# edouardoyallon/acco

Hardware: NVIDIA H100
Metric: tokens/sec (device-timed, max over ranks) Llama ACCO bf16 sharded-Adam, 8x1024 tokens per GPU per micro-batch (higher is better)
Workload: dtype bf16

## Files before the change

acco_b200/csrc/attention_wgmma.cu:

```cuda
#include <cuda.h>
#include <cuda_bf16.h>
#include <cuda_runtime.h>
#include <math.h>
#include <stdint.h>

#include "wgmma.cuh"

namespace acco_attn {

using namespace acco_tc;

constexpr int HD = 64;
constexpr int LDS = HD + 8;
constexpr float LOG2E = 1.4426950408889634f;
constexpr float LN2 = 0.6931471805599453f;

typedef __nv_bfloat16 bf16;

__device__ __forceinline__ uint32_t pack2(float a, float b) {
    __nv_bfloat162 h = __floats2bfloat162_rn(a, b);
    return *reinterpret_cast<uint32_t*>(&h);
}
__device__ __forceinline__ uint32_t ld32(const bf16* p) { return *reinterpret_cast<const uint32_t*>(p); }

__device__ __forceinline__ void mma16816(float (&c)[4], const uint32_t (&a)[4], uint32_t b0, uint32_t b1) {
    asm volatile("mma.sync.aligned.m16n8k16.row.col.f32.bf16.bf16.f32 {%0,%1,%2,%3}, {%4,%5,%6,%7}, {%8,%9}, {%0,%1,%2,%3};"
                 : "+f"(c[0]), "+f"(c[1]), "+f"(c[2]), "+f"(c[3])
                 : "r"(a[0]), "r"(a[1]), "r"(a[2]), "r"(a[3]), "r"(b0), "r"(b1));
}

template <int NB, int KB>
__device__ __forceinline__ void warp_mma_ss(float (&acc)[NB][4], const bf16* A, const bf16* B, int lane) {
    const int g = lane >> 2, t = lane & 3;
#pragma unroll
    for (int kb = 0; kb < KB; ++kb) {
        uint32_t a[4];
        const bf16* a0 = A + g * LDS + kb * 16 + 2 * t;
        a[0] = ld32(a0); a[1] = ld32(a0 + 8 * LDS); a[2] = ld32(a0 + 8); a[3] = ld32(a0 + 8 * LDS + 8);
#pragma unroll
        for (int nb = 0; nb < NB; ++nb) {
            const bf16* b = B + (nb * 8 + g) * LDS + kb * 16 + 2 * t;
            mma16816(acc[nb], a, ld32(b), ld32(b + 8));
        }
    }
}
template <int NB>
__device__ __forceinline__ void warp_mma_rs(float (&acc)[NB][4], const float (&p)[8][4], const bf16* B, int lane) {
    const int g = lane >> 2, t = lane & 3;
#pragma unroll
    for (int kb = 0; kb < 4; ++kb) {
        uint32_t a[4];
        a[0] = pack2(p[2 * kb][0], p[2 * kb][1]);
        a[1] = pack2(p[2 * kb][2], p[2 * kb][3]);
        a[2] = pack2(p[2 * kb + 1][0], p[2 * kb + 1][1]);
        a[3] = pack2(p[2 * kb + 1][2], p[2 * kb + 1][3]);
#pragma unroll
        for (int nb = 0; nb < NB; ++nb) {
            const bf16* b = B + (nb * 8 + g) * LDS + kb * 16 + 2 * t;
            mma16816(acc[nb], a, ld32(b), ld32(b + 8));
        }
    }
}

__device__ __forceinline__ void load_tile(bf16* dst, const bf16* src, long long ld, int rows, int valid, int tid, int nthr) {
    for (int i = tid; i < rows * 8; i += nthr) {
        const int r = i >> 3, c = (i & 7) * 8;
        uint4 v = make_uint4(0, 0, 0, 0);
        if (r < valid) v = *reinterpret_cast<const uint4*>(src + (long long)r * ld + c);
        *reinterpret_cast<uint4*>(dst + r * LDS + c) = v;
    }
}
__device__ __forceinline__ void load_tile_t(bf16* dst, const bf16* src, long long ld, int rows, int tid, int nthr) {
    for (int i = tid; i < rows * 8; i += nthr) {
        const int r = i >> 3, c = (i & 7) * 8;
        const uint4 v = *reinterpret_cast<const uint4*>(src + (long long)r * ld + c);
        const bf16* e = reinterpret_cast<const bf16*>(&v);
#pragma unroll
        for (int j = 0; j < 8; ++j) dst[(c + j) * LDS + r] = e[j];
    }
}

__device__ __forceinline__ bool visible(int q, int kv, int window) { return kv <= q && kv > q - window; }

struct FwdParams {
    CUtensorMap map_q;
    CUtensorMap map_k;
    CUtensorMap map_v;
    bf16* o;
    long long ld_o;
    float* lse;
    int B, S, Hq, Hk, window;
    float scale;
    const int* seg;
};

constexpr int FWD_Q = 128, FWD_KV = 64, FWD_THREADS = 256;
constexpr int FWD_TILE_KV = FWD_KV * HD * 2;
constexpr int FWD_SMEM = FWD_Q * HD * 2 + 2 * 2 * FWD_TILE_KV + 1024  + 64 ;

__device__ __forceinline__ void wgmma_m64n64k16_rs_tb(float (&d)[32], const uint32_t (&a)[4], uint64_t db) {
    asm volatile(
        "{\n\t.reg .pred p;\n\tsetp.ne.b32 p, %37, 0;\n\twgmma.mma_async.sync.aligned.m64n64k16.f32.bf16.bf16 "
        "{%0,%1,%2,%3,%4,%5,%6,%7,%8,%9,%10,%11,%12,%13,%14,%15,%16,%17,%18,%19,%20,%21,%22,%23,%24,%25,%26,%27,%28,%29,%30,%31}, "
        "{%32,%33,%34,%35}, %36, p, 1, 1, 1;\n\t}"
        : "+f"(d[0]), "+f"(d[1]), "+f"(d[2]), "+f"(d[3]), "+f"(d[4]), "+f"(d[5]), "+f"(d[6]), "+f"(d[7]), "+f"(d[8]), "+f"(d[9]), "+f"(d[10]),
          "+f"(d[11]), "+f"(d[12]), "+f"(d[13]), "+f"(d[14]), "+f"(d[15]), "+f"(d[16]), "+f"(d[17]), "+f"(d[18]), "+f"(d[19]), "+f"(d[20]),
          "+f"(d[21]), "+f"(d[22]), "+f"(d[23]), "+f"(d[24]), "+f"(d[25]), "+f"(d[26]), "+f"(d[27]), "+f"(d[28]), "+f"(d[29]), "+f"(d[30]),
          "+f"(d[31])
        : "r"(a[0]), "r"(a[1]), "r"(a[2]), "r"(a[3]), "l"(db), "r"(1));
}

template <bool kSeg>
__global__ void __launch_bounds__(FWD_THREADS) attn_fwd_kernel(const __grid_constant__ FwdParams P) {
    extern __shared__ uint8_t smem_raw[];
    uint8_t* smem = (uint8_t*)(((uintptr_t)smem_raw + 1023) & ~(uintptr_t)1023);
    uint8_t* sQ = smem;
    uint8_t* sKV = smem + FWD_Q * HD * 2;
    uint64_t* full = (uint64_t*)(sKV + 2 * 2 * FWD_TILE_KV);
    const int qb = blockIdx.x, h = blockIdx.y, b = blockIdx.z;
    const int hk = h / (P.Hq / P.Hk);
    const int tid = threadIdx.x, wg = tid >> 7, warp = (tid >> 5) & 3, lane = tid & 31, g = lane >> 2, t = lane & 3;
    const int q0 = qb * FWD_Q;
    const int row0 = b * P.S;
    int lo_key = max(0, q0 - P.window + 1);
    if constexpr (kSeg) lo_key = max(lo_key, P.seg[row0 + q0]);
    const int j_lo = lo_key / FWD_KV, j_hi = (q0 + FWD_Q - 1) / FWD_KV;
    auto issue = [&](int j) {
        const int s = (j - j_lo) & 1;
        mbar_expect_tx(&full[s], 2 * FWD_TILE_KV);
        tma_load_2d(&P.map_k, &full[s], sKV + s * 2 * FWD_TILE_KV, hk * HD, row0 + j * FWD_KV);
        tma_load_2d(&P.map_v, &full[s], sKV + s * 2 * FWD_TILE_KV + FWD_TILE_KV, hk * HD, row0 + j * FWD_KV);
    };
    if (tid == 0) {
        mbar_init(&full[0], 1);
        mbar_init(&full[1], 1);
        mbar_init(&full[2], 1);
        asm volatile("fence.mbarrier_init.release.cluster;" ::: "memory");
        mbar_expect_tx(&full[2], FWD_Q * HD * 2);
        tma_load_2d(&P.map_q, &full[2], sQ, h * HD, row0 + q0);
        issue(j_lo);
        if (j_lo + 1 <= j_hi) issue(j_lo + 1);
    }
    __syncthreads();
    mbar_wait(&full[2], 0);
    const float c = P.scale * LOG2E;
    float m_run[2] = {-INFINITY, -INFINITY}, l_run[2] = {0.f, 0.f};
    float o[32];
#pragma unroll
    for (int i = 0; i < 32; ++i) o[i] = 0.f;
    const int wq_lo = q0 + wg * 64, wq_hi = wq_lo + 63;
    const int qr[2] = {wq_lo + warp * 16 + g, wq_lo + warp * 16 + g + 8};
    int sg[2] = {0, 0}, wseg = 0;
    if constexpr (kSeg) {
        sg[0] = P.seg[row0 + qr[0]];
        sg[1] = P.seg[row0 + qr[1]];
        wseg = P.seg[row0 + wq_lo];
    }
    const uint32_t q_addr = smem_u32(sQ) + (uint32_t)(wg * 8192);
    for (int j = j_lo; j <= j_hi; ++j) {
        const int kv0 = j * FWD_KV, s = (j - j_lo) & 1;
        mbar_wait(&full[s], (uint32_t)(((j - j_lo) >> 1) & 1));
        if (!(kv0 > wq_hi || kv0 + FWD_KV - 1 <= wq_lo - P.window || (kSeg && kv0 + FWD_KV - 1 < wseg))) {
            const uint32_t k_addr = smem_u32(sKV + s * 2 * FWD_TILE_KV), v_addr = k_addr + FWD_TILE_KV;
            float sc[32];
#pragma unroll
            for (int i = 0; i < 32; ++i) sc[i] = 0.f;
            wgmma_fence();
#pragma unroll
            for (int k = 0; k < HD / 16; ++k)
                wgmma_m64n64k16<0, 0>(sc, make_smem_desc(q_addr + k * 32, 1, 1024 >> 4), make_smem_desc(k_addr + k * 32, 1, 1024 >> 4), 1u);
            wgmma_commit();
            wgmma_wait<0>();
            reg_fence(sc);
            float mx[2] = {-INFINITY, -INFINITY};
#pragma unroll
            for (int nb = 0; nb < 8; ++nb)
#pragma unroll
                for (int e = 0; e < 4; ++e) {
                    const int kv = kv0 + nb * 8 + 2 * t + (e & 1), r = e >> 1;
                    const float v = visible(qr[r], kv, P.window) && (!kSeg || kv >= sg[r]) ? sc[4 * nb + e] * c : -INFINITY;
                    sc[4 * nb + e] = v;
                    mx[r] = fmaxf(mx[r], v);
                }
#pragma unroll
            for (int r = 0; r < 2; ++r) {
                mx[r] = fmaxf(mx[r], __shfl_xor_sync(0xffffffffu, mx[r], 1));
                mx[r] = fmaxf(mx[r], __shfl_xor_sync(0xffffffffu, mx[r], 2));
            }
            float alpha[2], base[2], rs[2] = {0.f, 0.f};
#pragma unroll
            for (int r = 0; r < 2; ++r) {
                const float m_new = fmaxf(m_run[r], mx[r]);
                base[r] = m_new == -INFINITY ? 0.f : m_new;
                alpha[r] = exp2f(m_run[r] - base[r]);
                m_run[r] = m_new;
            }
#pragma unroll
            for (int i = 0; i < 32; ++i) {
                const int r = (i >> 1) & 1;
                const float p = exp2f(sc[i] - base[r]);
                sc[i] = p;
                rs[r] += p;
            }
#pragma unroll
            for (int r = 0; r < 2; ++r) {
                rs[r] += __shfl_xor_sync(0xffffffffu, rs[r], 1);
                rs[r] += __shfl_xor_sync(0xffffffffu, rs[r], 2);
                l_run[r] = l_run[r] * alpha[r] + rs[r];
            }
#pragma unroll
            for (int i = 0; i < 32; ++i) o[i] *= alpha[(i >> 1) & 1];
            wgmma_fence();
#pragma unroll
            for (int kk = 0; kk < FWD_KV / 16; ++kk) {
                uint32_t a[4];
                a[0] = pack2(sc[8 * kk + 0], sc[8 * kk + 1]);
                a[1] = pack2(sc[8 * kk + 2], sc[8 * kk + 3]);
                a[2] = pack2(sc[8 * kk + 4], sc[8 * kk + 5]);
                a[3] = pack2(sc[8 * kk + 6], sc[8 * kk + 7]);
                wgmma_m64n64k16_rs_tb(o, a, make_smem_desc(v_addr + kk * 2048, 8192 >> 4, 1024 >> 4));
            }
            wgmma_commit();
            wgmma_wait<0>();
            reg_fence(o);
        }
        __syncthreads();
        if (tid == 0 && j + 2 <= j_hi) issue(j + 2);
    }
#pragma unroll
    for (int r = 0; r < 2; ++r) {
        const int q = qr[r];
        const float inv = l_run[r] > 0.f ? 1.f / l_run[r] : 0.f;
        bf16* dst = P.o + ((long long)row0 + q) * P.ld_o + h * HD + 2 * t;
#pragma unroll
        for (int nb = 0; nb < 8; ++nb)
            *reinterpret_cast<uint32_t*>(dst + nb * 8) = pack2(o[4 * nb + 2 * r] * inv, o[4 * nb + 2 * r + 1] * inv);
        if (t == 0) P.lse[((long long)b * P.Hq + h) * P.S + q] = (m_run[r] + log2f(l_run[r])) * LN2;
    }
}

struct BwdParams {
    const bf16 *q, *k, *v;
    long long ld;
    const bf16* d_o;
    long long ld_do;
    const float *lse, *delta;
    float* dq;
    bf16 *dk, *dv;
    int B, S, Hq, Hk, window;
    float scale;
    const int* seg;
};

constexpr int BWD_KV = 64, BWD_Q = 64, BWD_THREADS = 128;
constexpr int BWD_SMEM = 8 * 64 * LDS * 2 + 2 * BWD_Q * 4;
constexpr int BWD_SMEM_SEG = BWD_SMEM + (BWD_Q + 1) * 4;

template <bool kSeg>
__global__ void __launch_bounds__(BWD_THREADS) attn_bwd_kernel(const BwdParams P) {
    extern __shared__ __align__(16) uint8_t smem_raw[];
    bf16* sK = reinterpret_cast<bf16*>(smem_raw);
    bf16* sKt = sK + 64 * LDS;
    bf16* sV = sKt + 64 * LDS;
    bf16* sQ = sV + 64 * LDS;
    bf16* sQt = sQ + 64 * LDS;
    bf16* sdO = sQt + 64 * LDS;
    bf16* sdOt = sdO + 64 * LDS;
    bf16* sdS = sdOt + 64 * LDS;
    float* sL = reinterpret_cast<float*>(sdS + 64 * LDS);
    float* sD = sL + BWD_Q;
    int* sSeg = reinterpret_cast<int*>(sD + BWD_Q);
    const int nb_k = blockIdx.x, hk = blockIdx.y, b = blockIdx.z;
    const int G = P.Hq / P.Hk;
    const int tid = threadIdx.x, warp = tid >> 5, lane = tid & 31, g = lane >> 2, t = lane & 3;
    const int kv0 = nb_k * BWD_KV;
    const long long row0 = (long long)b * P.S;
    load_tile(sK, P.k + (row0 + kv0) * P.ld + hk * HD, P.ld, BWD_KV, BWD_KV, tid, BWD_THREADS);
    load_tile_t(sKt, P.k + (row0 + kv0) * P.ld + hk * HD, P.ld, BWD_KV, tid, BWD_THREADS);
    load_tile(sV, P.v + (row0 + kv0) * P.ld + hk * HD, P.ld, BWD_KV, BWD_KV, tid, BWD_THREADS);
    const float c = P.scale * LOG2E;
    float dk[8][4], dv[8][4];
#pragma unroll
    for (int i = 0; i < 8; ++i)
#pragma unroll
        for (int e = 0; e < 4; ++e) dk[i][e] = dv[i][e] = 0.f;
    const int kr[2] = {kv0 + warp * 16 + g, kv0 + warp * 16 + g + 8};
    const int m_lo = kv0 / BWD_Q;
    const int m_hi = min(P.S / BWD_Q - 1, (kv0 + BWD_KV - 1 + P.window - 1) / BWD_Q);
    for (int gi = 0; gi < G; ++gi) {
        const int hq = hk * G + gi;
        for (int m = m_lo; m <= m_hi; ++m) {
            const int q0 = m * BWD_Q;
            __syncthreads();
            load_tile(sQ, P.q + (row0 + q0) * P.ld + hq * HD, P.ld, BWD_Q, BWD_Q, tid, BWD_THREADS);
            load_tile_t(sQt, P.q + (row0 + q0) * P.ld + hq * HD, P.ld, BWD_Q, tid, BWD_THREADS);
            load_tile(sdO, P.d_o + (row0 + q0) * P.ld_do + hq * HD, P.ld_do, BWD_Q, BWD_Q, tid, BWD_THREADS);
            load_tile_t(sdOt, P.d_o + (row0 + q0) * P.ld_do + hq * HD, P.ld_do, BWD_Q, tid, BWD_THREADS);
            if (tid < BWD_Q) {
                const long long li = ((long long)b * P.Hq + hq) * P.S + q0 + tid;
                sL[tid] = P.lse[li] * LOG2E;
                sD[tid] = P.delta[li];
                if constexpr (kSeg) sSeg[tid] = P.seg[row0 + q0 + tid];
            }
            if (kSeg && tid == BWD_Q) sSeg[BWD_Q] = m == m_hi || P.seg[row0 + q0 + BWD_Q] > kv0 + BWD_KV - 1;
            __syncthreads();
            float s[8][4], dp[8][4];
#pragma unroll
            for (int i = 0; i < 8; ++i)
#pragma unroll
                for (int e = 0; e < 4; ++e) s[i][e] = dp[i][e] = 0.f;
            warp_mma_ss<8, 4>(s, sK + warp * 16 * LDS, sQ, lane);
            warp_mma_ss<8, 4>(dp, sV + warp * 16 * LDS, sdO, lane);
#pragma unroll
            for (int nb = 0; nb < 8; ++nb)
#pragma unroll
                for (int e = 0; e < 4; ++e) {
                    const int ql = nb * 8 + 2 * t + (e & 1), q = q0 + ql, r = e >> 1;
                    const float p = visible(q, kr[r], P.window) && (!kSeg || kr[r] >= sSeg[ql]) ? exp2f(s[nb][e] * c - sL[ql]) : 0.f;
                    const float pb = __bfloat162float(__float2bfloat16(p));
                    s[nb][e] = pb;
                    dp[nb][e] = __bfloat162float(__float2bfloat16(p * (dp[nb][e] - sD[ql]) * P.scale));
                }
#pragma unroll
            for (int nb = 0; nb < 8; ++nb)
#pragma unroll
                for (int e = 0; e < 4; ++e) {
                    const int ql = nb * 8 + 2 * t + (e & 1), kl = warp * 16 + g + 8 * (e >> 1);
                    sdS[ql * LDS + kl] = __float2bfloat16(dp[nb][e]);
                }
            warp_mma_rs<8>(dv, s, sdOt, lane);
            warp_mma_rs<8>(dk, dp, sQt, lane);
            __syncthreads();
            float dq[8][4];
#pragma unroll
            for (int i = 0; i < 8; ++i) dq[i][0] = dq[i][1] = dq[i][2] = dq[i][3] = 0.f;
            warp_mma_ss<8, 4>(dq, sdS + warp * 16 * LDS, sKt, lane);
#pragma unroll
            for (int r = 0; r < 2; ++r) {
                float* dst = P.dq + (row0 + q0 + warp * 16 + g + 8 * r) * (long long)(P.Hq * HD) + hq * HD + 2 * t;
#pragma unroll
                for (int nb = 0; nb < 8; ++nb) {
                    atomicAdd(dst + nb * 8, dq[nb][2 * r]);
                    atomicAdd(dst + nb * 8 + 1, dq[nb][2 * r + 1]);
                }
            }
            if (kSeg && sSeg[BWD_Q]) break;
        }
    }
#pragma unroll
    for (int r = 0; r < 2; ++r) {
        const long long off = (row0 + kr[r]) * (long long)(P.Hk * HD) + hk * HD + 2 * t;
#pragma unroll
        for (int nb = 0; nb < 8; ++nb) {
            *reinterpret_cast<uint32_t*>(P.dk + off + nb * 8) = pack2(dk[nb][2 * r], dk[nb][2 * r + 1]);
            *reinterpret_cast<uint32_t*>(P.dv + off + nb * 8) = pack2(dv[nb][2 * r], dv[nb][2 * r + 1]);
        }
    }
}

__global__ void __launch_bounds__(256) attn_delta_kernel(const bf16* __restrict__ o, const bf16* __restrict__ d_o, long long ld_o,
                                                         long long ld_do, float* __restrict__ delta, int B, int S, int Hq) {
    const long long item = ((long long)blockIdx.x * blockDim.x + threadIdx.x) >> 3;
    const int part = threadIdx.x & 7;
    const long long n_items = (long long)B * S * Hq;
    float acc = 0.f;
    long long row = 0;
    int h = 0;
    if (item < n_items) {
        row = item / Hq;
        h = (int)(item - row * Hq);
        const uint4 a = *reinterpret_cast<const uint4*>(o + row * ld_o + h * HD + part * 8);
        const uint4 d = *reinterpret_cast<const uint4*>(d_o + row * ld_do + h * HD + part * 8);
        const __nv_bfloat162* a2 = reinterpret_cast<const __nv_bfloat162*>(&a);
        const __nv_bfloat162* d2 = reinterpret_cast<const __nv_bfloat162*>(&d);
#pragma unroll
        for (int i = 0; i < 4; ++i) {
            const float2 x = __bfloat1622float2(a2[i]), y = __bfloat1622float2(d2[i]);
            acc += x.x * y.x + x.y * y.y;
        }
    }
    acc += __shfl_xor_sync(0xffffffffu, acc, 1);
    acc += __shfl_xor_sync(0xffffffffu, acc, 2);
    acc += __shfl_xor_sync(0xffffffffu, acc, 4);
    if (item < n_items && part == 0) {
        const long long b = row / S, s = row - b * S;
        delta[(b * Hq + h) * S + s] = acc;
    }
}

static bool shape_ok(int B, int S, int Hq, int Hk, int D, float scale) {
    return B > 0 && S > 0 && S % 128 == 0 && Hk > 0 && Hq > 0 && Hq % Hk == 0 && D == HD && scale > 0.f;
}
static bool aligned(const void* p, long long ld) { return ((uintptr_t)p % 16) == 0 && (ld % 8) == 0; }
static int eff_window(int S, int window) { return (window <= 0 || window > S) ? S : window; }

}

extern "C" int acco_attn_supported(int B, int S, int Hq, int Hk, int D, float scale) {
    return acco_attn::shape_ok(B, S, Hq, Hk, D, scale) ? 1 : 0;
}

extern "C" int acco_attn_fwd(const void* q, const void* k, const void* v, long long ld, void* o, long long ld_o, float* lse, int B, int S, int Hq,
                             int Hk, int D, float scale, int window, const int* seg, cudaStream_t st) {
    using namespace acco_attn;
    if (!shape_ok(B, S, Hq, Hk, D, scale) || !aligned(q, ld) || !aligned(k, ld) || !aligned(v, ld) || !aligned(o, ld_o)) return -1;
    static int fwd_attr = (int)cudaFuncSetAttribute(attn_fwd_kernel<false>, cudaFuncAttributeMaxDynamicSharedMemorySize, FWD_SMEM);
    static int fwd_attr_seg = (int)cudaFuncSetAttribute(attn_fwd_kernel<true>, cudaFuncAttributeMaxDynamicSharedMemorySize, FWD_SMEM);
    if (fwd_attr) return fwd_attr;
    if (fwd_attr_seg) return fwd_attr_seg;
    FwdParams P;
    const uint64_t rows = (uint64_t)B * S;
    int rc = acco_gemm::make_map_typed(&P.map_q, q, (uint64_t)Hq * HD, rows, (uint64_t)ld, HD, FWD_Q, 2);
    if (!rc) rc = acco_gemm::make_map_typed(&P.map_k, k, (uint64_t)Hk * HD, rows, (uint64_t)ld, HD, FWD_KV, 2);
    if (!rc) rc = acco_gemm::make_map_typed(&P.map_v, v, (uint64_t)Hk * HD, rows, (uint64_t)ld, HD, FWD_KV, 2);
    if (rc) return rc;
    P.o = (bf16*)o; P.ld_o = ld_o; P.lse = lse;
    P.B = B; P.S = S; P.Hq = Hq; P.Hk = Hk; P.window = eff_window(S, window); P.scale = scale; P.seg = seg;
    if (seg)
        attn_fwd_kernel<true><<<dim3(S / FWD_Q, Hq, B), FWD_THREADS, FWD_SMEM, st>>>(P);
    else
        attn_fwd_kernel<false><<<dim3(S / FWD_Q, Hq, B), FWD_THREADS, FWD_SMEM, st>>>(P);
    return (int)cudaGetLastError();
}

extern "C" int acco_attn_bwd(const void* q, const void* k, const void* v, long long ld, const void* o, long long ld_o, const void* d_o,
                             long long ld_do, const float* lse, float* delta, float* dq_acc, void* dk, void* dv, int B, int S, int Hq, int Hk, int D,
                             float scale, int window, const int* seg, cudaStream_t st) {
    using namespace acco_attn;
    if (!shape_ok(B, S, Hq, Hk, D, scale) || !aligned(q, ld) || !aligned(k, ld) || !aligned(v, ld) || !aligned(o, ld_o) || !aligned(d_o, ld_do))
        return -1;
    static int attr_rc = (int)cudaFuncSetAttribute(attn_bwd_kernel<false>, cudaFuncAttributeMaxDynamicSharedMemorySize, BWD_SMEM);
    static int attr_rc_seg = (int)cudaFuncSetAttribute(attn_bwd_kernel<true>, cudaFuncAttributeMaxDynamicSharedMemorySize, BWD_SMEM_SEG);
    if (attr_rc) return attr_rc;
    if (attr_rc_seg) return attr_rc_seg;
    const long long items = (long long)B * S * Hq;
    attn_delta_kernel<<<(unsigned)((items * 8 + 255) / 256), 256, 0, st>>>((const bf16*)o, (const bf16*)d_o, ld_o, ld_do, delta, B, S, Hq);
    if (cudaMemsetAsync(dq_acc, 0, (size_t)items * HD * sizeof(float), st) != cudaSuccess) return -6;
    BwdParams P{(const bf16*)q, (const bf16*)k, (const bf16*)v, ld, (const bf16*)d_o, ld_do, lse, delta, dq_acc, (bf16*)dk, (bf16*)dv,
                B, S, Hq, Hk, eff_window(S, window), scale, seg};
    if (seg)
        attn_bwd_kernel<true><<<dim3(S / BWD_KV, Hk, B), BWD_THREADS, BWD_SMEM_SEG, st>>>(P);
    else
        attn_bwd_kernel<false><<<dim3(S / BWD_KV, Hk, B), BWD_THREADS, BWD_SMEM, st>>>(P);
    return (int)cudaGetLastError();
}
```

acco_b200/csrc/wgmma.cuh:

```cuda
#pragma once
#include <cuda.h>
#include <cuda_bf16.h>
#include <cuda_runtime.h>
#include <stdint.h>
#include <stdio.h>

namespace acco_tc {

__device__ __forceinline__ uint32_t smem_u32(const void* p) { return (uint32_t)__cvta_generic_to_shared(p); }

__device__ __forceinline__ void mbar_init(uint64_t* bar, uint32_t count) {
    asm volatile("mbarrier.init.shared::cta.b64 [%0], %1;" ::"r"(smem_u32(bar)), "r"(count));
}
__device__ __forceinline__ void mbar_expect_tx(uint64_t* bar, uint32_t bytes) {
    asm volatile("mbarrier.arrive.expect_tx.shared::cta.b64 _, [%0], %1;" ::"r"(smem_u32(bar)), "r"(bytes) : "memory");
}
__device__ __forceinline__ void mbar_arrive(uint64_t* bar) {
    asm volatile("mbarrier.arrive.shared::cta.b64 _, [%0];" ::"r"(smem_u32(bar)) : "memory");
}
__device__ __forceinline__ void mbar_wait(uint64_t* bar, uint32_t parity) {
    uint32_t done = 0;
    unsigned spins = 0;
    unsigned long long t0 = 0;
    const uint32_t addr = smem_u32(bar);
    while (true) {
        asm volatile(
            "{\n\t"
            ".reg .pred p;\n\t"
            "mbarrier.try_wait.parity.shared::cta.b64 p, [%1], %2;\n\t"
            "selp.u32 %0, 1, 0, p;\n\t"
            "}"
            : "=r"(done)
            : "r"(addr), "r"(parity)
            : "memory");
        if (done) break;
        if ((++spins & 0x3FFF) == 0) {
            unsigned long long now;
            asm volatile("mov.u64 %0, %%globaltimer;" : "=l"(now));
            if (t0 == 0) t0 = now;
            else if (now - t0 > 20ull * 1000000000ull) __trap();
        }
    }
}
__device__ __forceinline__ void tma_load_2d(const CUtensorMap* map, uint64_t* bar, void* smem, int c0, int c1) {
    asm volatile(
        "cp.async.bulk.tensor.2d.shared::cluster.global.mbarrier::complete_tx::bytes [%0], [%1, {%3, %4}], [%2];" ::"r"(
            smem_u32(smem)),
        "l"(map), "r"(smem_u32(bar)), "r"(c0), "r"(c1)
        : "memory");
}
__device__ __forceinline__ void tma_load_2d_mc(const CUtensorMap* map, uint64_t* bar, void* smem, int c0, int c1, uint16_t mask) {
    asm volatile(
        "cp.async.bulk.tensor.2d.shared::cluster.global.mbarrier::complete_tx::bytes.multicast::cluster [%0], [%1, {%3, %4}], [%2], %5;" ::"r"(
            smem_u32(smem)),
        "l"(map), "r"(smem_u32(bar)), "r"(c0), "r"(c1), "h"(mask)
        : "memory");
}
__device__ __forceinline__ void tma_store_2d(const CUtensorMap* map, const void* smem, int c0, int c1) {
    asm volatile("cp.async.bulk.tensor.2d.global.shared::cta.bulk_group [%0, {%2, %3}], [%1];" ::"l"(map), "r"(smem_u32(smem)),
                 "r"(c0), "r"(c1)
                 : "memory");
}
__device__ __forceinline__ void tma_reduce_add_2d(const CUtensorMap* map, const void* smem, int c0, int c1) {
    asm volatile("cp.reduce.async.bulk.tensor.2d.global.shared::cta.add.tile.bulk_group [%0, {%2, %3}], [%1];" ::"l"(map),
                 "r"(smem_u32(smem)), "r"(c0), "r"(c1)
                 : "memory");
}
__device__ __forceinline__ void bulk_commit() { asm volatile("cp.async.bulk.commit_group;" ::: "memory"); }
template <int N>
__device__ __forceinline__ void bulk_wait_read() { asm volatile("cp.async.bulk.wait_group.read %0;" ::"n"(N) : "memory"); }
template <int N>
__device__ __forceinline__ void bulk_wait() { asm volatile("cp.async.bulk.wait_group %0;" ::"n"(N) : "memory"); }
__device__ __forceinline__ uint32_t cluster_ctarank() {
    uint32_t r;
    asm volatile("mov.u32 %0, %%cluster_ctarank;" : "=r"(r));
    return r;
}
__device__ __forceinline__ void cluster_sync_all() {
    asm volatile("barrier.cluster.arrive.release.aligned;" ::: "memory");
    asm volatile("barrier.cluster.wait.acquire.aligned;" ::: "memory");
}
__device__ __forceinline__ uint32_t map_to_cta(const void* smem_ptr, uint32_t cta) {
    uint32_t remote;
    asm volatile("mapa.shared::cluster.u32 %0, %1, %2;" : "=r"(remote) : "r"(smem_u32(smem_ptr)), "r"(cta));
    return remote;
}
__device__ __forceinline__ void mbar_arrive_cluster_addr(uint32_t addr) {
    asm volatile("mbarrier.arrive.release.cluster.shared::cluster.b64 _, [%0];" ::"r"(addr) : "memory");
}
__device__ __forceinline__ void fence_async_smem() { asm volatile("fence.proxy.async.shared::cta;" ::: "memory"); }

__device__ __forceinline__ uint64_t make_smem_desc(uint32_t smem_addr, uint32_t lbo, uint32_t sbo) {
    uint64_t d = 0;
    d |= (uint64_t)((smem_addr & 0x3FFFF) >> 4);
    d |= (uint64_t)(lbo & 0x3FFF) << 16;
    d |= (uint64_t)(sbo & 0x3FFF) << 32;
    d |= (uint64_t)1 << 62;
    return d;
}
__device__ __forceinline__ void wgmma_fence() { asm volatile("wgmma.fence.sync.aligned;" ::: "memory"); }
__device__ __forceinline__ void wgmma_commit() { asm volatile("wgmma.commit_group.sync.aligned;" ::: "memory"); }
template <int N>
__device__ __forceinline__ void wgmma_wait() { asm volatile("wgmma.wait_group.sync.aligned %0;" ::"n"(N) : "memory"); }
template <int R>
__device__ __forceinline__ void reg_fence(float (&d)[R]) {
#pragma unroll
    for (int i = 0; i < R; ++i) asm volatile("" : "+f"(d[i])::"memory");
}
__device__ __forceinline__ void named_barrier(int id, int threads) { asm volatile("bar.sync %0, %1;" ::"r"(id), "r"(threads) : "memory"); }
__device__ __forceinline__ uint32_t ld_shared_u32(uint32_t addr) {
    uint32_t v;
    asm volatile("ld.shared.u32 %0, [%1];" : "=r"(v) : "r"(addr) : "memory");
    return v;
}
__device__ __forceinline__ void st_shared_u32(uint32_t addr, uint32_t v) { asm volatile("st.shared.u32 [%0], %1;" ::"r"(addr), "r"(v) : "memory"); }
__device__ __forceinline__ uint32_t pack_bf16x2(float a, float b) {
    __nv_bfloat162 h = __floats2bfloat162_rn(a, b);
    return *reinterpret_cast<uint32_t*>(&h);
}

__device__ __forceinline__ uint4 pack_bf16x8(const float* f) {
    uint4 pk;
    __nv_bfloat162 h0 = __floats2bfloat162_rn(f[0], f[1]);
    __nv_bfloat162 h1 = __floats2bfloat162_rn(f[2], f[3]);
    __nv_bfloat162 h2 = __floats2bfloat162_rn(f[4], f[5]);
    __nv_bfloat162 h3 = __floats2bfloat162_rn(f[6], f[7]);
    pk.x = *reinterpret_cast<uint32_t*>(&h0);
    pk.y = *reinterpret_cast<uint32_t*>(&h1);
    pk.z = *reinterpret_cast<uint32_t*>(&h2);
    pk.w = *reinterpret_cast<uint32_t*>(&h3);
    return pk;
}

// ... 67 lines not shown
```

Before: 384,700.

## Rewrite attention backward with TMA producer warp, mbarrier pipeline, and WGMMA

```diff
diff --git a/acco_b200/csrc/attention_wgmma.cu b/acco_b200/csrc/attention_wgmma.cu
--- a/acco_b200/csrc/attention_wgmma.cu
+++ b/acco_b200/csrc/attention_wgmma.cu
@@ -11,7 +11,6 @@
 using namespace acco_tc;
 
 constexpr int HD = 64;
-constexpr int LDS = HD + 8;
 constexpr float LOG2E = 1.4426950408889634f;
 constexpr float LN2 = 0.6931471805599453f;
 
@@ -21,65 +20,6 @@
     __nv_bfloat162 h = __floats2bfloat162_rn(a, b);
     return *reinterpret_cast<uint32_t*>(&h);
 }
-__device__ __forceinline__ uint32_t ld32(const bf16* p) { return *reinterpret_cast<const uint32_t*>(p); }
-
-__device__ __forceinline__ void mma16816(float (&c)[4], const uint32_t (&a)[4], uint32_t b0, uint32_t b1) {
-    asm volatile("mma.sync.aligned.m16n8k16.row.col.f32.bf16.bf16.f32 {%0,%1,%2,%3}, {%4,%5,%6,%7}, {%8,%9}, {%0,%1,%2,%3};"
-                 : "+f"(c[0]), "+f"(c[1]), "+f"(c[2]), "+f"(c[3])
-                 : "r"(a[0]), "r"(a[1]), "r"(a[2]), "r"(a[3]), "r"(b0), "r"(b1));
-}
-
-template <int NB, int KB>
-__device__ __forceinline__ void warp_mma_ss(float (&acc)[NB][4], const bf16* A, const bf16* B, int lane) {
-    const int g = lane >> 2, t = lane & 3;
-#pragma unroll
-    for (int kb = 0; kb < KB; ++kb) {
-        uint32_t a[4];
-        const bf16* a0 = A + g * LDS + kb * 16 + 2 * t;
-        a[0] = ld32(a0); a[1] = ld32(a0 + 8 * LDS); a[2] = ld32(a0 + 8); a[3] = ld32(a0 + 8 * LDS + 8);
-#pragma unroll
-        for (int nb = 0; nb < NB; ++nb) {
-            const bf16* b = B + (nb * 8 + g) * LDS + kb * 16 + 2 * t;
-            mma16816(acc[nb], a, ld32(b), ld32(b + 8));
-        }
-    }
-}
-template <int NB>
-__device__ __forceinline__ void warp_mma_rs(float (&acc)[NB][4], const float (&p)[8][4], const bf16* B, int lane) {
-    const int g = lane >> 2, t = lane & 3;
-#pragma unroll
-    for (int kb = 0; kb < 4; ++kb) {
-        uint32_t a[4];
-        a[0] = pack2(p[2 * kb][0], p[2 * kb][1]);
-        a[1] = pack2(p[2 * kb][2], p[2 * kb][3]);
-        a[2] = pack2(p[2 * kb + 1][0], p[2 * kb + 1][1]);
-        a[3] = pack2(p[2 * kb + 1][2], p[2 * kb + 1][3]);
-#pragma unroll
-        for (int nb = 0; nb < NB; ++nb) {
-            const bf16* b = B + (nb * 8 + g) * LDS + kb * 16 + 2 * t;
-            mma16816(acc[nb], a, ld32(b), ld32(b + 8));
-        }
-    }
-}
-
-__device__ __forceinline__ void load_tile(bf16* dst, const bf16* src, long long ld, int rows, int valid, int tid, int nthr) {
-    for (int i = tid; i < rows * 8; i += nthr) {
-        const int r = i >> 3, c = (i & 7) * 8;
-        uint4 v = make_uint4(0, 0, 0, 0);
-        if (r < valid) v = *reinterpret_cast<const uint4*>(src + (long long)r * ld + c);
-        *reinterpret_cast<uint4*>(dst + r * LDS + c) = v;
-    }
-}
-__device__ __forceinline__ void load_tile_t(bf16* dst, const bf16* src, long long ld, int rows, int tid, int nthr) {
-    for (int i = tid; i < rows * 8; i += nthr) {
-        const int r = i >> 3, c = (i & 7) * 8;
-        const uint4 v = *reinterpret_cast<const uint4*>(src + (long long)r * ld + c);
-        const bf16* e = reinterpret_cast<const bf16*>(&v);
-#pragma unroll
-        for (int j = 0; j < 8; ++j) dst[(c + j) * LDS + r] = e[j];
-    }
-}
-
 __device__ __forceinline__ bool visible(int q, int kv, int window) { return kv <= q && kv > q - window; }
 
 struct FwdParams {
@@ -240,10 +180,10 @@
 }
 
 struct BwdParams {
-    const bf16 *q, *k, *v;
-    long long ld;
-    const bf16* d_o;
-    long long ld_do;
+    CUtensorMap map_q;
+    CUtensorMap map_k;
+    CUtensorMap map_v;
+    CUtensorMap map_do;
     const float *lse, *delta;
     float* dq;
     bf16 *dk, *dv;
@@ -252,108 +192,159 @@
     const int* seg;
 };
 
-constexpr int BWD_KV = 64, BWD_Q = 64, BWD_THREADS = 128;
-constexpr int BWD_SMEM = 8 * 64 * LDS * 2 + 2 * BWD_Q * 4;
-constexpr int BWD_SMEM_SEG = BWD_SMEM + (BWD_Q + 1) * 4;
+constexpr int BWD_KV = 64, BWD_Q = 64, BWD_STAGES = 2;
+constexpr int BWD_THREADS = 160;
+constexpr int BWD_TILE = 64 * HD * 2;
+constexpr int BWD_VEC = 3 * BWD_Q * 4;
+constexpr int BWD_SMEM = (3 + 2 * BWD_STAGES) * BWD_TILE + BWD_STAGES * BWD_VEC + 1024  + 64 ;
 
 template <bool kSeg>
-__global__ void __launch_bounds__(BWD_THREADS) attn_bwd_kernel(const BwdParams P) {
-    extern __shared__ __align__(16) uint8_t smem_raw[];
-    bf16* sK = reinterpret_cast<bf16*>(smem_raw);
-    bf16* sKt = sK + 64 * LDS;
-    bf16* sV = sKt + 64 * LDS;
-    bf16* sQ = sV + 64 * LDS;
-    bf16* sQt = sQ + 64 * LDS;
-    bf16* sdO = sQt + 64 * LDS;
-    bf16* sdOt = sdO + 64 * LDS;
-    bf16* sdS = sdOt + 64 * LDS;
-    float* sL = reinterpret_cast<float*>(sdS + 64 * LDS);
-    float* sD = sL + BWD_Q;
-    int* sSeg = reinterpret_cast<int*>(sD + BWD_Q);
+__global__ void __launch_bounds__(BWD_THREADS, 2) attn_bwd_kernel(const __grid_constant__ BwdParams P) {
+    extern __shared__ uint8_t smem_raw[];
+    uint8_t* smem = (uint8_t*)(((uintptr_t)smem_raw + 1023) & ~(uintptr_t)1023);
+    uint8_t* sK = smem;
+    uint8_t* sV = smem + BWD_TILE;
+    uint8_t* sdS = smem + 2 * BWD_TILE;
+    uint8_t* sQdO = smem + 3 * BWD_TILE;
+    float* sVec = (float*)(smem + (3 + 2 * BWD_STAGES) * BWD_TILE);
+    uint64_t* full = (uint64_t*)(sVec + BWD_STAGES * 3 * BWD_Q);
+    uint64_t* empty = full + BWD_STAGES;
+    uint64_t* kv_full = empty + BWD_STAGES;
     const int nb_k = blockIdx.x, hk = blockIdx.y, b = blockIdx.z;
     const int G = P.Hq / P.Hk;
-    const int tid = threadIdx.x, warp = tid >> 5, lane = tid & 31, g = lane >> 2, t = lane & 3;
+    const int tid = threadIdx.x;
     const int kv0 = nb_k * BWD_KV;
-    const long long row0 = (long long)b * P.S;
-    load_tile(sK, P.k + (row0 + kv0) * P.ld + hk * HD, P.ld, BWD_KV, BWD_KV, tid, BWD_THREADS);
-    load_tile_t(sKt, P.k + (row0 + kv0) * P.ld + hk * HD, P.ld, BWD_KV, tid, BWD_THREADS);
-    load_tile(sV, P.v + (row0 + kv0) * P.ld + hk * HD, P.ld, BWD_KV, BWD_KV, tid, BWD_THREADS);
+    const int row0 = b * P.S;
+    const int m_lo = kv0 / BWD_Q;
+    int m_end = min(P.S / BWD_Q - 1, (kv0 + BWD_KV - 1 + P.window - 1) / BWD_Q) + 1;
+    if constexpr (kSeg) {
+        int m = m_lo + 1;
+        while (m < m_end && P.seg[row0 + m * BWD_Q] <= kv0 + BWD_KV - 1) ++m;
+        m_end = m;
+    }
+    const int nm = m_end - m_lo, n_it = G * nm;
+    if (tid == 0) {
+        for (int s = 0; s < BWD_STAGES; ++s) {
+            mbar_init(&full[s], 1);
+            mbar_init(&empty[s], 128);
+        }
+        mbar_init(kv_full, 1);
+        asm volatile("fence.mbarrier_init.release.cluster;" ::: "memory");
+    }
+    __syncthreads();
+    if (__shfl_sync(0xffffffffu, tid >> 5, 0) == 4) {
+        if (tid == 128) {
+            mbar_expect_tx(kv_full, 2 * BWD_TILE);
+            tma_load_2d(&P.map_k, kv_full, sK, hk * HD, row0 + kv0);
+            tma_load_2d(&P.map_v, kv_full, sV, hk * HD, row0 + kv0);
+            for (int i = 0; i < n_it; ++i) {
+                const int s = i % BWD_STAGES, hq = hk * G + i / nm, q0 = (m_lo + i % nm) * BWD_Q;
+                if (i >= BWD_STAGES) mbar_wait(&empty[s], (uint32_t)((i / BWD_STAGES - 1) & 1));
+                const long long li = ((long long)b * P.Hq + hq) * P.S + q0;
+                float* vec = sVec + s * 3 * BWD_Q;
+                mbar_expect_tx(&full[s], 2 * BWD_TILE + (kSeg ? 3 : 2) * BWD_Q * 4);
+                tma_load_2d(&P.map_q, &full[s], sQdO + 2 * s * BWD_TILE, hq * HD, row0 + q0);
+                tma_load_2d(&P.map_do, &full[s], sQdO + (2 * s + 1) * BWD_TILE, hq * HD, row0 + q0);
+                bulk_load(vec, P.lse + li, BWD_Q * 4, &full[s]);
+                bulk_load(vec + BWD_Q, P.delta + li, BWD_Q * 4, &full[s]);
+                if constexpr (kSeg) bulk_load(vec + 2 * BWD_Q, P.seg + row0 + q0, BWD_Q * 4, &full[s]);
+            }
+        }
+        return;
+    }
+    const int warp = tid >> 5, lane = tid & 31, g = lane >> 2, t = lane & 3;
     const float c = P.scale * LOG2E;
-    float dk[8][4], dv[8][4];
-#pragma unroll
-    for (int i = 0; i < 8; ++i)
-#pragma unroll
-        for (int e = 0; e < 4; ++e) dk[i][e] = dv[i][e] = 0.f;
+    float dk[32], dv[32];
+#pragma unroll
+    for (int i = 0; i < 32; ++i) dk[i] = dv[i] = 0.f;
     const int kr[2] = {kv0 + warp * 16 + g, kv0 + warp * 16 + g + 8};
-    const int m_lo = kv0 / BWD_Q;
-    const int m_hi = min(P.S / BWD_Q - 1, (kv0 + BWD_KV - 1 + P.window - 1) / BWD_Q);
-    for (int gi = 0; gi < G; ++gi) {
-        const int hq = hk * G + gi;
-        for (int m = m_lo; m <= m_hi; ++m) {
-            const int q0 = m * BWD_Q;
-            __syncthreads();
-            load_tile(sQ, P.q + (row0 + q0) * P.ld + hq * HD, P.ld, BWD_Q, BWD_Q, tid, BWD_THREADS);
-            load_tile_t(sQt, P.q + (row0 + q0) * P.ld + hq * HD, P.ld, BWD_Q, tid, BWD_THREADS);
-            load_tile(sdO, P.d_o + (row0 + q0) * P.ld_do + hq * HD, P.ld_do, BWD_Q, BWD_Q, tid, BWD_THREADS);
-            load_tile_t(sdOt, P.d_o + (row0 + q0) * P.ld_do + hq * HD, P.ld_do, BWD_Q, tid, BWD_THREADS);
-            if (tid < BWD_Q) {
-                const long long li = ((long long)b * P.Hq + hq) * P.S + q0 + tid;
-                sL[tid] = P.lse[li] * LOG2E;
-                sD[tid] = P.delta[li];
-                if constexpr (kSeg) sSeg[tid] = P.seg[row0 + q0 + tid];
-            }
-            if (kSeg && tid == BWD_Q) sSeg[BWD_Q] = m == m_hi || P.seg[row0 + q0 + BWD_Q] > kv0 + BWD_KV - 1;
-            __syncthreads();
-            float s[8][4], dp[8][4];
-#pragma unroll
-            for (int i = 0; i < 8; ++i)
-#pragma unroll
-                for (int e = 0; e < 4; ++e) s[i][e] = dp[i][e] = 0.f;
-            warp_mma_ss<8, 4>(s, sK + warp * 16 * LDS, sQ, lane);
-            warp_mma_ss<8, 4>(dp, sV + warp * 16 * LDS, sdO, lane);
-#pragma unroll
-            for (int nb = 0; nb < 8; ++nb)
-#pragma unroll
-                for (int e = 0; e < 4; ++e) {
-                    const int ql = nb * 8 + 2 * t + (e & 1), q = q0 + ql, r = e >> 1;
-                    const float p = visible(q, kr[r], P.window) && (!kSeg || kr[r] >= sSeg[ql]) ? exp2f(s[nb][e] * c - sL[ql]) : 0.f;
-                    const float pb = __bfloat162float(__float2bfloat16(p));
-                    s[nb][e] = pb;
-                    dp[nb][e] = __bfloat162float(__float2bfloat16(p * (dp[nb][e] - sD[ql]) * P.scale));
+    const uint32_t k_addr = smem_u32(sK), v_addr = smem_u32(sV), ds_addr = smem_u32(sdS);
+    mbar_wait(kv_full, 0);
+    for (int i = 0; i < n_it; ++i) {
+        const int s = i % BWD_STAGES, hq = hk * G + i / nm, q0 = (m_lo + i % nm) * BWD_Q;
+        const uint32_t q_addr = smem_u32(sQdO + 2 * s * BWD_TILE), do_addr = q_addr + BWD_TILE;
+        const float* lse = sVec + s * 3 * BWD_Q;
+        const float* delta = lse + BWD_Q;
+        const int* sg = reinterpret_cast<const int*>(lse + 2 * BWD_Q);
+        mbar_wait(&full[s], (uint32_t)((i / BWD_STAGES) & 1));
+        float st[32], dpt[32];
+#pragma unroll
+        for (int e = 0; e < 32; ++e) st[e] = dpt[e] = 0.f;
+        wgmma_fence();
+#pragma unroll
+        for (int k = 0; k < HD / 16; ++k)
+            wgmma_m64n64k16<0, 0>(st, make_smem_desc(k_addr + k * 32, 1, 1024 >> 4), make_smem_desc(q_addr + k * 32, 1, 1024 >> 4), 1u);
+#pragma unroll
+        for (int k = 0; k < HD / 16; ++k)
+            wgmma_m64n64k16<0, 0>(dpt, make_smem_desc(v_addr + k * 32, 1, 1024 >> 4), make_smem_desc(do_addr + k * 32, 1, 1024 >> 4), 1u);
+        wgmma_commit();
+        wgmma_wait<0>();
+        reg_fence(st);
+        reg_fence(dpt);
+        const bool need_mask = kSeg || q0 < kv0 + BWD_KV - 1 || q0 + BWD_Q - 1 - P.window >= kv0;
+        uint32_t pa[16], dsa[16];
+#pragma unroll
+        for (int nb = 0; nb < 8; ++nb) {
+            const int ql = nb * 8 + 2 * t;
+            const float2 L = *reinterpret_cast<const float2*>(lse + ql);
+            const float2 Dl = *reinterpret_cast<const float2*>(delta + ql);
+#pragma unroll
+            for (int h = 0; h < 2; ++h) {
+                float p[2], d[2];
+#pragma unroll
+                for (int j = 0; j < 2; ++j) {
+                    const int e = 4 * nb + 2 * h + j;
+                    float pv = exp2f(st[e] * c - (j ? L.y : L.x) * LOG2E);
+                    if (need_mask && !(visible(q0 + ql + j, kr[h], P.window) && (!kSeg || kr[h] >= sg[ql + j]))) pv = 0.f;
+                    p[j] = pv;
+                    d[j] = pv * (dpt[e] - (j ? Dl.y : Dl.x)) * P.scale;
                 }
-#pragma unroll
-            for (int nb = 0; nb < 8; ++nb)
-#pragma unroll
-                for (int e = 0; e < 4; ++e) {
-                    const int ql = nb * 8 + 2 * t + (e & 1), kl = warp * 16 + g + 8 * (e >> 1);
-                    sdS[ql * LDS + kl] = __float2bfloat16(dp[nb][e]);
-                }
-            warp_mma_rs<8>(dv, s, sdOt, lane);
-            warp_mma_rs<8>(dk, dp, sQt, lane);
-            __syncthreads();
-            float dq[8][4];
-#pragma unroll
-            for (int i = 0; i < 8; ++i) dq[i][0] = dq[i][1] = dq[i][2] = dq[i][3] = 0.f;
-            warp_mma_ss<8, 4>(dq, sdS + warp * 16 * LDS, sKt, lane);
-#pragma unroll
-            for (int r = 0; r < 2; ++r) {
-                float* dst = P.dq + (row0 + q0 + warp * 16 + g + 8 * r) * (long long)(P.Hq * HD) + hq * HD + 2 * t;
-#pragma unroll
-                for (int nb = 0; nb < 8; ++nb) {
-                    atomicAdd(dst + nb * 8, dq[nb][2 * r]);
-                    atomicAdd(dst + nb * 8 + 1, dq[nb][2 * r + 1]);
-                }
-            }
-            if (kSeg && sSeg[BWD_Q]) break;
-        }
-    }
-#pragma unroll
-    for (int r = 0; r < 2; ++r) {
-        const long long off = (row0 + kr[r]) * (long long)(P.Hk * HD) + hk * HD + 2 * t;
+                pa[2 * nb + h] = pack2(p[0], p[1]);
+                dsa[2 * nb + h] = pack2(d[0], d[1]);
+                st_shared_u32(ds_addr + (uint32_t)((warp * 16 + g + 8 * h) * 128 + ((nb ^ g) << 4) + 4 * t), dsa[2 * nb + h]);
+            }
+        }
+        fence_async_smem();
+        float dqa[32];
+#pragma unroll
+        for (int e = 0; e < 32; ++e) dqa[e] = 0.f;
+        wgmma_fence();
+#pragma unroll
+        for (int kk = 0; kk < BWD_Q / 16; ++kk) {
+            const uint32_t a[4] = {pa[4 * kk], pa[4 * kk + 1], pa[4 * kk + 2], pa[4 * kk + 3]};
+            wgmma_m64n64k16_rs_tb(dv, a, make_smem_desc(do_addr + kk * 2048, 8192 >> 4, 1024 >> 4));
+        }
+#pragma unroll
+        for (int kk = 0; kk < BWD_Q / 16; ++kk) {
+            const uint32_t a[4] = {dsa[4 * kk], dsa[4 * kk + 1], dsa[4 * kk + 2], dsa[4 * kk + 3]};
+            wgmma_m64n64k16_rs_tb(dk, a, make_smem_desc(q_addr + kk * 2048, 8192 >> 4, 1024 >> 4));
+        }
+        wgmma_commit();
+        named_barrier(1, 128);
+#pragma unroll
+        for (int kk = 0; kk < BWD_KV / 16; ++kk)
+            wgmma_m64n64k16<1, 1>(dqa, make_smem_desc(ds_addr + kk * 2048, 8192 >> 4, 1024 >> 4),
+                                  make_smem_desc(k_addr + kk * 2048, 8192 >> 4, 1024 >> 4), 1u);
+        wgmma_commit();
+        wgmma_wait<0>();
+        reg_fence(dv);
+        reg_fence(dk);
+        reg_fence(dqa);
+        mbar_arrive(&empty[s]);
+#pragma unroll
+        for (int h = 0; h < 2; ++h) {
+            float* dst = P.dq + ((long long)row0 + q0 + warp * 16 + g + 8 * h) * (long long)(P.Hq * HD) + hq * HD + 2 * t;
+#pragma unroll
+            for (int nb = 0; nb < 8; ++nb) atomicAdd(reinterpret_cast<float2*>(dst + nb * 8), make_float2(dqa[4 * nb + 2 * h], dqa[4 * nb + 2 * h + 1]));
+        }
+    }
+#pragma unroll
+    for (int h = 0; h < 2; ++h) {
+        const long long off = ((long long)row0 + kr[h]) * (long long)(P.Hk * HD) + hk * HD + 2 * t;
 #pragma unroll
         for (int nb = 0; nb < 8; ++nb) {
-            *reinterpret_cast<uint32_t*>(P.dk + off + nb * 8) = pack2(dk[nb][2 * r], dk[nb][2 * r + 1]);
-            *reinterpret_cast<uint32_t*>(P.dv + off + nb * 8) = pack2(dv[nb][2 * r], dv[nb][2 * r + 1]);
+            *reinterpret_cast<uint32_t*>(P.dk + off + nb * 8) = pack2(dk[4 * nb + 2 * h], dk[4 * nb + 2 * h + 1]);
+            *reinterpret_cast<uint32_t*>(P.dv + off + nb * 8) = pack2(dv[4 * nb + 2 * h], dv[4 * nb + 2 * h + 1]);
         }
     }
 }
@@ -427,19 +418,27 @@
                              long long ld_do, const float* lse, float* delta, float* dq_acc, void* dk, void* dv, int B, int S, int Hq, int Hk, int D,
                              float scale, int window, const int* seg, cudaStream_t st) {
     using namespace acco_attn;
-    if (!shape_ok(B, S, Hq, Hk, D, scale) || !aligned(q, ld) || !aligned(k, ld) || !aligned(v, ld) || !aligned(o, ld_o) || !aligned(d_o, ld_do))
+    if (!shape_ok(B, S, Hq, Hk, D, scale) || !aligned(q, ld) || !aligned(k, ld) || !aligned(v, ld) || !aligned(o, ld_o) || !aligned(d_o, ld_do) ||
+        !aligned(lse, 0) || !aligned(delta, 0) || (seg && !aligned(seg, 0)))
         return -1;
     static int attr_rc = (int)cudaFuncSetAttribute(attn_bwd_kernel<false>, cudaFuncAttributeMaxDynamicSharedMemorySize, BWD_SMEM);
-    static int attr_rc_seg = (int)cudaFuncSetAttribute(attn_bwd_kernel<true>, cudaFuncAttributeMaxDynamicSharedMemorySize, BWD_SMEM_SEG);
+    static int attr_rc_seg = (int)cudaFuncSetAttribute(attn_bwd_kernel<true>, cudaFuncAttributeMaxDynamicSharedMemorySize, BWD_SMEM);
     if (attr_rc) return attr_rc;
     if (attr_rc_seg) return attr_rc_seg;
     const long long items = (long long)B * S * Hq;
     attn_delta_kernel<<<(unsigned)((items * 8 + 255) / 256), 256, 0, st>>>((const bf16*)o, (const bf16*)d_o, ld_o, ld_do, delta, B, S, Hq);
     if (cudaMemsetAsync(dq_acc, 0, (size_t)items * HD * sizeof(float), st) != cudaSuccess) return -6;
-    BwdParams P{(const bf16*)q, (const bf16*)k, (const bf16*)v, ld, (const bf16*)d_o, ld_do, lse, delta, dq_acc, (bf16*)dk, (bf16*)dv,
-                B, S, Hq, Hk, eff_window(S, window), scale, seg};
+    BwdParams P;
+    const uint64_t rows = (uint64_t)B * S;
+    int rc = acco_gemm::make_map_typed(&P.map_q, q, (uint64_t)Hq * HD, rows, (uint64_t)ld, HD, BWD_Q, 2);
+    if (!rc) rc = acco_gemm::make_map_typed(&P.map_k, k, (uint64_t)Hk * HD, rows, (uint64_t)ld, HD, BWD_KV, 2);
+    if (!rc) rc = acco_gemm::make_map_typed(&P.map_v, v, (uint64_t)Hk * HD, rows, (uint64_t)ld, HD, BWD_KV, 2);
+    if (!rc) rc = acco_gemm::make_map_typed(&P.map_do, d_o, (uint64_t)Hq * HD, rows, (uint64_t)ld_do, HD, BWD_Q, 2);
+    if (rc) return rc;
+    P.lse = lse; P.delta = delta; P.dq = dq_acc; P.dk = (bf16*)dk; P.dv = (bf16*)dv;
+    P.B = B; P.S = S; P.Hq = Hq; P.Hk = Hk; P.window = eff_window(S, window); P.scale = scale; P.seg = seg;
     if (seg)
-        attn_bwd_kernel<true><<<dim3(S / BWD_KV, Hk, B), BWD_THREADS, BWD_SMEM_SEG, st>>>(P);
+        attn_bwd_kernel<true><<<dim3(S / BWD_KV, Hk, B), BWD_THREADS, BWD_SMEM, st>>>(P);
     else
         attn_bwd_kernel<false><<<dim3(S / BWD_KV, Hk, B), BWD_THREADS, BWD_SMEM, st>>>(P);
     return (int)cudaGetLastError();
diff --git a/acco_b200/csrc/wgmma.cuh b/acco_b200/csrc/wgmma.cuh
--- a/acco_b200/csrc/wgmma.cuh
+++ b/acco_b200/csrc/wgmma.cuh
@@ -49,6 +49,11 @@
         "l"(map), "r"(smem_u32(bar)), "r"(c0), "r"(c1)
         : "memory");
 }
+__device__ __forceinline__ void bulk_load(void* smem, const void* gmem, uint32_t bytes, uint64_t* bar) {
+    asm volatile("cp.async.bulk.shared::cluster.global.mbarrier::complete_tx::bytes [%0], [%1], %2, [%3];" ::"r"(smem_u32(smem)), "l"(gmem),
+                 "r"(bytes), "r"(smem_u32(bar))
+                 : "memory");
+}
 __device__ __forceinline__ void tma_load_2d_mc(const CUtensorMap* map, uint64_t* bar, void* smem, int c0, int c1, uint16_t mask) {
     asm volatile(
         "cp.async.bulk.tensor.2d.shared::cluster.global.mbarrier::complete_tx::bytes.multicast::cluster [%0], [%1, {%3, %4}], [%2], %5;" ::"r"(
```

New measurement: 385,400, median of 6. No clear change (+0.2%).
